# hihixuyang/LQR-Obstacles

Hardware: AMD Instinct MI355X
Metric: agent-pair LQR-obstacle evals/sec (higher is better)
Workload: dtype f64

## Files before the change

lqr-obstacles_amd/csrc/lqro_device.hpp:

```cpp
#pragma once
#include <hip/hip_runtime.h>
#include <stdint.h>

namespace lqro {

constexpr int kWave = 64;

#define LQRO_ROW_BIG (1 << 20)

#define LQRO_ST_PAIRS 0
#define LQRO_ST_PLANES 1
#define LQRO_ST_INSIDE 2
#define LQRO_ST_HULLOK 3
#define LQRO_ST_HULLFAIL 4
#define LQRO_ST_BACKUP 5
#define LQRO_ST_NREACH 6
#define LQRO_ST_GTESTS 7
#define LQRO_ST_MERGED 8
#define LQRO_ST_RETRY 9
#define LQRO_ST_TIMEOUT 10
#define LQRO_ST_NFAIL 11
#define LQRO_ST_MWIN 12
#define LQRO_ST_NBUILD 13
#define LQRO_ST_FAILS 16
// ... 14 lines not shown
  LQRO_HC_HOT = 6,
  LQRO_HC_HOT_NEXT = 7,
  LQRO_HC_UNUSED8 = 8,
  LQRO_HC_LP4 = 9,
  LQRO_HC_LP4_NEXT = 10,
  LQRO_HC_LHAND = 11,
  LQRO_HC_LHAND_NEXT = 12,
  LQRO_HC_LDONE = 13,
  LQRO_HC_UNUSED14 = 14,
  LQRO_HC_FACET0 = 15,
  LQRO_HC_WORDS = 16
};

enum : int {
  LQRO_H2_PREV = 0,
  LQRO_H2_HOT1 = 1,
  LQRO_H2_HOT1_NEXT = 2,
  LQRO_H2_HOT2_NEXT = 3,
  LQRO_H2_HOT2_DONE = 4,
  LQRO_H2_SPEC = 5,
  LQRO_H2_SPEC_NEXT = 6,
  LQRO_H2_UNUSED7 = 7,
  LQRO_H2_WORDS = 8
};

enum : int {
  LQRO_PROF_HULL = 0,
  LQRO_PROF_HJOBS = LQRO_PROF_HULL + 32,
  LQRO_PROF_PAIR = LQRO_PROF_HJOBS + 2 * 4096,
  LQRO_PROF_LFAIL = LQRO_PROF_PAIR + 16 + 16,
  LQRO_PROF_LJOBS = LQRO_PROF_LFAIL + 16,
  LQRO_PROF_QW1 = LQRO_PROF_LJOBS + 4 * 4096,
  LQRO_PROF_QLONG = LQRO_PROF_QW1 + 64,
  LQRO_PROF_WORDS = LQRO_PROF_QLONG + 24 * 1024,
  LQRO_PROF_HULL_WORDS = LQRO_PROF_LFAIL
};

__device__ __forceinline__ int opaque(int x) {
  asm volatile("" : "+v"(x));
  return x;
}

__device__ __forceinline__ double uniform(double v) {
  const long long b = __double_as_longlong(v);
  const int lo = __builtin_amdgcn_readfirstlane((int)b);
  const int hi = __builtin_amdgcn_readfirstlane((int)(b >> 32));
  return __longlong_as_double(((long long)hi << 32) | (unsigned)lo);
}

__device__ __forceinline__ void wave_lds_sync() {
  __builtin_amdgcn_fence(__ATOMIC_RELEASE, "workgroup");
  __builtin_amdgcn_wave_barrier();
  __builtin_amdgcn_fence(__ATOMIC_ACQUIRE, "workgroup");
}

template <int CTRL, int ROWS>
__device__ __forceinline__ int dpp_i(int old, int x) {
  return __builtin_amdgcn_update_dpp(old, x, CTRL, ROWS, 0xF, false);
}
template <int CTRL, int ROWS>
__device__ __forceinline__ double dpp_d(double old, double x) {
  const long long o = __double_as_longlong(old), v = __double_as_longlong(x);
  const int lo = dpp_i<CTRL, ROWS>((int)o, (int)v);
  const int hi = dpp_i<CTRL, ROWS>((int)(o >> 32), (int)(v >> 32));
  return __longlong_as_double(((long long)hi << 32) | (unsigned)lo);
}
__device__ __forceinline__ int wave_incl_scan(int x) {
// ... 107 lines not shown
```

lqr-obstacles_amd/csrc/lqro_plan.hpp:

```cpp
#pragma once

#include <algorithm>
#include <climits>
#include <cstddef>
#include <cstdlib>
#include <vector>

namespace lqro {

struct StepKnobs {
  int hot_on;
  int hot_split;
  int hot_spec;
  long hot_max_inside;
  double hot_t, hot_r;
  int qside;
  int qside_pct;
  int qspare;
  int qbalance;
  int qhull_inline;
  int qhull_big;
  int qhull_flags;
  int hull_big_only;
  int local_hull;
// ... 5 lines not shown

inline int env_int(const char* name, int dflt) {
  const char* e = std::getenv(name);
  return e ? std::atoi(e) : dflt;
}
inline long env_long(const char* name, long dflt) {
  const char* e = std::getenv(name);
  return e ? std::atol(e) : dflt;
}
inline double env_double(const char* name, double dflt) {
  const char* e = std::getenv(name);
  return e ? std::atof(e) : dflt;
}

inline StepKnobs knobs_from_env(int n_cu) {
  StepKnobs k{};
  k.qhull_big = env_int("LQRO_QHULL_BIG", 0) != 0;
  k.side_cus = std::max(0, std::min(n_cu / 2, env_int("LQRO_SIDE_HULL_CUS", (3 * n_cu) / 8)));
  k.hull_big_only = env_int("LQRO_HULL_BIG", 0) != 0;
  k.local_hull = env_int("LQRO_LOCAL_HULL", 1) != 0;
  k.lside_cus = std::max(0, std::min(n_cu / 2, env_int("LQRO_LOCAL_SIDE_CUS", (3 * n_cu) / 16)));
  k.hot_on = env_int("LQRO_HOT", 1) != 0;
  k.hot_t = env_double("LQRO_HOT_T", 3.0);
  k.hot_r = env_double("LQRO_HOT_R", 3.0);
  k.lhull_prof = env_int("LQRO_LHULL_PROFILE", 0) != 0;
  k.hot_max_inside = env_long("LQRO_HOT_MAX_INSIDE", -1L);
  k.early_lp = env_int("LQRO_EARLY_LP", 1) != 0;
  k.hot_split = env_int("LQRO_HOT_SPLIT", 1) != 0;
  k.hot_spec = env_int("LQRO_HOT_SPEC", 1) != 0;
  k.qspare = env_int("LQRO_QHULL_SPARE", 4);
  k.qside_pct = std::max(1, std::min(100, env_int("LQRO_QHULL_SIDE_PCT", 100)));
  k.qside = env_int("LQRO_QSIDE", 0) != 0;
  k.qhull_inline = env_int("LQRO_QHULL_INLINE_BIG", 1) != 0;
  k.qhull_flags = env_int("LQRO_QHULL_FLAGS", 119);
  k.qbalance = env_int("LQRO_QHULL_BALANCE", 1) != 0;
  return k;
}

struct StepFeedback {
  unsigned long long inside;
  unsigned long long sweep_work;
  unsigned long long build_work;
  unsigned long long build_max;
  unsigned long long retried;
  unsigned long long unused[3];
};
static_assert(sizeof(StepFeedback) == 8 * sizeof(unsigned long long), "one slot is 8 words");
constexpr StepFeedback kNoFeedback = {~0ull, 0ull, 0ull, 0ull, 0ull, {0ull, 0ull, 0ull}};

struct StepShape {
  int n_cu, nrows;
  int npr;
  int nbr_k;
  size_t hnp;
  int per_agent, qhull_order;
  int phase;
  bool has_newv;
  bool newv_is_callers;
  int waves, lds_wave, wave_doubles;
  size_t hull_lds_max_hnp;
  size_t hull_lds_doubles;
  int hull_cwaves;
  size_t qhull_lds_doubles;
  size_t lp_lds_max;
  int early_lp_max_npr;
  int row_big;
  int extra_planes = 0;
// ... 135 lines not shown
```

lqr-obstacles_amd/csrc/lqro_qh_front.inc:

```
int simplex[4];
{
  int maxpoints[6];
  S.max_outside = 0.0;
  S.MAXabs_coord = 0.0;
  S.MAXwidth = -DBL_MAX;
  S.MAXsumcoord = 0.0;
  for (int k = 0; k < 3; k++) {
    int mn, mx;
    qh_extreme(W.Pr, n, k, false, lane, &mn);
    qh_extreme(W.Pr, n, k, true, lane, &mx);
    const double maxk = W.Pr[3 * (size_t)mx + k], mink = W.Pr[3 * (size_t)mn + k];
    const double maxcoord = fmax(maxk, -mink);
    const double temp = maxk - mink;
    if (temp > S.MAXwidth) S.MAXwidth = temp;
    if (maxcoord > S.MAXabs_coord) S.MAXabs_coord = maxcoord;
    S.MAXsumcoord += maxcoord;
    maxpoints[2 * k] = mn;
    maxpoints[2 * k + 1] = mx;
    S.NEARzero[k] = 80 * S.MAXsumcoord * DBL_EPSILON;
  }
  {
    double maxdistsum = sqrt(3.0) * S.MAXabs_coord;
    if (S.MAXsumcoord < maxdistsum) maxdistsum = S.MAXsumcoord;
    S.DISTround = DBL_EPSILON * (3 * maxdistsum * 1.01 + S.MAXabs_coord);
    const double MINdenom_1 = fmax(1.0 / DBL_MAX, DBL_MIN);
    S.MINdenom = MINdenom_1 * S.MAXabs_coord;
    S.MINdenom_2 = sqrt(MINdenom_1 * 3) * S.MAXabs_coord;
    S.MINvisible = 0.0 + 2 * S.DISTround;
    S.MAXcoplanar = S.MINvisible;
    S.MINoutside = 2 * S.MINvisible;
  }
  {
    double maxcoord = -DBL_MAX, mincoord = DBL_MAX;
    int minx = -1, maxx = -1;
    for (int i = 0; i < 6; i++) {
      const double c = W.Pr[3 * (size_t)maxpoints[i]];
      if (maxcoord < c) { maxcoord = c; maxx = maxpoints[i]; }
      if (mincoord > c) { mincoord = c; minx = maxpoints[i]; }
    }
    double maxdet = maxcoord - mincoord;
    int ns = 0;
    simplex[ns++] = minx;
    if (maxx != minx) simplex[ns++] = maxx;
    if (ns < 2) { S.status |= QHS_INPUT; QH_FRONT_FAIL; }
    for (int i = 2; i < 4; i++) {
      const double prevdet = maxdet;
      int maxpoint = -1, maxnearzero = 0, nearzero;
      maxdet = -1.0;
      for (int m = 0; m < 6; m++) {
        const int p = maxpoints[m];
        bool ins = false;
        for (int t = 0; t < i; t++) ins |= simplex[t] == p;
        if (!ins && p != maxpoint) {
// ... 30 lines not shown
```

lqr-obstacles_amd/csrc/lqro_qhull3.hpp:

```cpp
#pragma once
#include "lqro_qhull.hpp"
#include "lqro_qhull3_prof.hpp"
#include "lqro_lp.hpp"

namespace lqro {

#ifndef Q3_NEWCAP
#define Q3_NEWCAP 128
#endif
#ifndef Q3_VISCAP
#define Q3_VISCAP 192
#endif
#define Q3_MOVCAP 16
#define Q3_HZCAP 24
#define Q3_COPCAP 8
#define Q3_FSTK 512
#define Q3_ND (Q3_NEWCAP + Q3_MOVCAP)
#define Q3_WAVES 4
#define Q3_HR 4
#ifndef Q3_W0_SLEEP
#define Q3_W0_SLEEP 1
#endif
#ifndef Q3_W1_SLEEP
#define Q3_W1_SLEEP 1
// ... 1686 lines not shown
    int cnt = 0;
    if (vi < nvis) {
      const int f = L.sp_visf[vi];
      cnt = (int)(q3_cc(W, L, f) & 0xffffu) - (vi == 0 ? 1 : 0);
      L.pf_vsoff[vi] = W.soff[f];
      L.pf_vscnt[vi] = cnt;
    }
    np += __builtin_amdgcn_readlane(q3_scan_add(cnt), 63);
  }
  hl_sync();
  if (lane < np) {
    int a = 0, base = 0;
    for (;;) {
      const int k = L.pf_vscnt[a];
      if (lane < base + k || a == nvis - 1) break;
      base += k;
      ++a;
    }
    const int q = W.sb[L.pf_vsoff[a] + lane - base];
    HullPt r;
    r.x = W.Pr[3 * (size_t)q]; r.y = W.Pr[3 * (size_t)q + 1]; r.z = W.Pr[3 * (size_t)q + 2];
    r.q = q;
    r.pad = 0;
    L.pf_pre[lane] = r;
    L.pf_prea[lane] = (unsigned char)a;
  }
  hl_sync();
  if (lane == 0) {
    L.pf_np = np;
    q3_st_rel(&L.pf_done, p);
  }
}

__device__ inline void q3_build(const Q3W& W, Q3S& S, Q3L& L, int n, int lane) {
#ifdef LQRO_QHULL_PROFILE
  S.pf.tq = __builtin_amdgcn_s_memtime();
#endif
  const unsigned long long ltmask = (1ull << lane) - 1ull;
  S.status = 0;
  S.nalloc = 1;
  S.nfs = 0;
  S.sbtop = 0;
  S.nnew = S.nvis = S.nmov = S.nold = 0;
  S.findbestnew = S.notsharp = 0;
  S.hgen = 0;
  S.egen = 0;
  S.keyc = 1;
  S.key0_last = 0;
  S.qhead = S.qtail = 0;
  if (W.FC > 65535) {
    S.status |= QHS_CAPACITY | Q3_CAPBIT(QHS_CAP_FACETS);
    return;
  }
#define QH_FRONT_FAIL return
#include "lqro_qh_front.inc"
#undef QH_FRONT_FAIL
  const int pset[4] = {simplex[3], simplex[2], simplex[1], simplex[0]};
  int fs[4];
  {
    int top = 1, tops[4];
    for (int i = 0; i < 4; i++) {
      fs[i] = S.nalloc++;
      tops[i] = top;
      top ^= 1;
    }
    for (int k = 0; k < 3; k++) {
      double c = 0.0;
      for (int t = 0; t < 4; t++) c += W.Pr[3 * (size_t)pset[t] + k];
      S.interior[k] = c / 4;
    }
    int fv[4][3];
    for (int i = 0; i < 4; i++) {
      int m = 0;
      for (int t = 0; t < 4; t++)
        if (t != i) fv[i][m++] = pset[t];
    }
    int ls = 0;
    double q[4][4];
    bool fl[4];
    q3_plane(S, ls, W.Pr + 3 * (size_t)fv[0][0], W.Pr + 3 * (size_t)fv[0][1], W.Pr + 3 * (size_t)fv[0][2], tops[0],
             q[0], &fl[0]);
    if (q3_distq(q[0], S.interior) > S.DISTround)
      for (int i = 0; i < 4; i++) tops[i] ^= 1;
    bool anyflip = false;
    for (int i = 0; i < 4; i++) {
      q3_plane(S, ls, W.Pr + 3 * (size_t)fv[i][0], W.Pr + 3 * (size_t)fv[i][1], W.Pr + 3 * (size_t)fv[i][2],
               tops[i], q[i], &fl[i]);
      anyflip |= fl[i];
    }
    if (anyflip) ls |= QHS_FLIPPED;
    int nbs[4][3];
    for (int i = 0; i < 4; i++) {
      int m = 0;
      for (int t = 0; t < 4; t++)
        if (t != i) nbs[i][m++] = fs[t];
    }
    double minangle = DBL_MAX;
    for (int i = 0; i < 4; i++)
      for (int t = 0; t < 3; t++) {
        int j = 0;
        for (int u = 0; u < 4; u++)
          if (fs[u] == nbs[i][t]) j = u;
        double angle = 0.0;
        for (int k = 0; k < 3; k++) angle += q[i][k] * q[j][k];
        if (angle < minangle) minangle = angle;
      }
    if (minangle < -0.99999999) ls |= QHS_NARROW;
    S.status |= ls;
    hl_sync();
    if (lane == 0)
      for (int i = 0; i < 4; i++) {
        const int f = fs[i];
        q3_set_facet(W, L, f, q[i], nbs[i][0], nbs[i][1], nbs[i][2],
                     QF_LIVE | (tops[i] ? QF_TOP : 0) | (fl[i] ? QF_FLIPPED : 0));
        q3_set_key(W, L, f, S.keyc + i);
        q3_set_cc(W, L, f, 0u);
        Q3V& v = W.vv[f];
        for (int t = 0; t < 3; t++) {
          for (int k = 0; k < 3; k++) v.p[3 * t + k] = W.Pr[3 * (size_t)fv[i][t] + k];
          v.id[t] = fv[i][t];
        }
      }
    S.keyc += 4;
    hl_sync();
    int np = 0;
    for (int c = 0; c < n; c += 64) {
      const int qi = c + lane;
      const bool ok = qi < n && qi != simplex[0] && qi != simplex[1] && qi != simplex[2] && qi != simplex[3];
      const unsigned long long b = __ballot(ok);
      if (ok) W.pq[np + __popcll(b & ltmask)] = qi;
      np += __popcll(b);
    }
    hl_sync();
    const double distoutside = fmax(2 * S.MINoutside, S.max_outside);
    for (int i = 0; i < 4; i++) {
      const int f = fs[i];
      int cnt = 0;
      const int off = S.sbtop;
      double mx = 0.0, cx = 0.0, cy = 0.0, cz = 0.0;
      int champ = -1, w = 0;
      for (int c = 0; c < np; c += 64) {
        const int pos = c + lane;
        HullPt pt;
        pt.x = pt.y = pt.z = 0.0;
        pt.q = -1;
        pt.pad = 0;
        double d = -DBL_MAX;
        if (pos < np) {
          pt.q = W.pq[pos];
          pt.x = W.Pr[3 * (size_t)pt.q]; pt.y = W.Pr[3 * (size_t)pt.q + 1]; pt.z = W.Pr[3 * (size_t)pt.q + 2];
          const double p[3] = {pt.x, pt.y, pt.z};
          d = q3_distq(q[i], p);
        }
        const bool out = pos < np && d >= distoutside;
        const bool keep = pos < np && !out;
        const unsigned long long bk = __ballot(keep);
        hl_sync();
        if (keep) W.pq[w + __popcll(bk & ltmask)] = pt.q;
        w += __popcll(bk);
        const unsigned long long bo = __ballot(out);
        if (bo) {
          int wpos = -1, wr = 0;
          q3_place(bo, lane, ltmask, d, pt, off, W.SB, cnt, mx, champ, cx, cy, cz, wpos, wr);
          if (wpos >= 0) W.sb[wpos] = wr;
        }
        hl_sync();
      }
      if (cnt) {
        if (off + cnt > W.SB) { S.status |= QHS_CAPACITY | Q3_CAPBIT(QHS_CAP_SB); return; }
        if (lane == 0) {
          W.sb[off + cnt - 1] = champ;
          W.soff[f] = off;
          W.fdist[f] = mx;
          q3_set_cc(W, L, f, (unsigned)cnt | ((unsigned)champ << 16));
        }
        S.sbtop += cnt;
      }
      np = w;
      hl_sync();
    }
    if (np > 0) {
      S.nnew = 4;
      if (lane == 0)
        for (int i = 0; i < 4; i++) {
          L.nslot[i] = fs[i];
          for (int k = 0; k < 4; k++) L.npl[4 * i + k] = q[i][k];
          L.nflag[i] = q3_fa(W, L, fs[i]);
          L.nn1[i] = L.nn2[i] = 0;
        }
      S.nmov = 0;
      S.findbestnew = 1;
      hl_sync();
      int rg;
      double rd;
      HullPt rpt, pre;
      pre.x = pre.y = pre.z = 0.0;
      pre.q = -1;
      pre.pad = 0;
      q3_locate_seq(W, S, L, np, 0, true, lane, pre, 0, false, rg, rd, rpt);
      q3_emit_seq(W, S, L, np, 0, true, lane, rg, rd, rpt);
      S.findbestnew = 0;
      S.nnew = 0;
      S.nmov = 0;
      hl_sync();
    }
    if (S.status & (QHS_INPUT | QHS_TOPOLOGY | QHS_CAPACITY)) return;
    {
      int order[4] = {fs[0], fs[1], fs[2], fs[3]};
      unsigned kk[4];
      for (int i = 0; i < 4; i++) kk[i] = q3_key(W, L, order[i]);
      for (int a = 0; a < 4; a++)
        for (int b = a + 1; b < 4; b++)
          if (kk[b] < kk[a]) {
            const unsigned tk = kk[a]; kk[a] = kk[b]; kk[b] = tk;
            const int to = order[a]; order[a] = order[b]; order[b] = to;
          }
      int best = -1;
      double bd = -DBL_MAX;
      for (int i = 0; i < 4; i++) {
        const int f = order[i];
        if ((q3_cc(W, L, f) & 0xffffu) && W.fdist[f] > bd) { best = f; bd = W.fdist[f]; }
      }
      hl_sync();
      if (best >= 0) {
        q3_set_key(W, L, best, 0u);
        for (int i = 0; i < 4; i++)
          if (order[i] == best) {
            for (int t = i; t > 0; t--) { order[t] = order[t - 1]; kk[t] = kk[t - 1]; }
            order[0] = best;
            kk[0] = 0;
            break;
          }
      }
      int qt = 0;
      for (int i = 0; i < 4; i++)
        if (q3_cc(W, L, order[i]) & 0xffffu) {
          if (lane == 0) {
            W.fq[qt] = order[i];
            W.fqk[qt] = kk[i];
            HullPt r;
            r.x = r.y = r.z = 0.0; r.q = -1; r.pad = 0;
            W.fqc[qt] = r;
          }
          qt++;
        }
      S.qhead = 0;
      S.qtail = qt;
      hl_sync();
    }
  }
  Q3T(0);
  if (lane == 0) {
    L.c_dist[0] = S.MINvisible; L.c_dist[1] = S.MAXcoplanar; L.c_dist[2] = S.DISTround;
    L.c_dist[3] = S.MINdenom; L.c_dist[4] = S.MINdenom_2;
    for (int k = 0; k < 3; k++) { L.c_dist[5 + k] = S.NEARzero[k]; L.c_interior[k] = S.interior[k]; }
  }
  int phase = 0;
  int qcb = 0, qcn = 0;
  int qf = 0, qp = -1;
  unsigned qk = 0;
  double qx = 0.0, qy = 0.0, qz = 0.0;
  for (;;) {
#ifdef LQRO_QHULL_PROFILE
    unsigned long long snap_[21];
    for (int k = 0; k < 21; k++) snap_[k] = S.pf.tph[k];
#endif
    int facet = -1, furthest = -1;
    double apexp[3] = {0.0, 0.0, 0.0};
    bool adopt = false;
    bool pfv = false;
    bool fast = false;
    int nvis = 0, nnew = 0, lm = 0;
    const double* ncb = W.ncoord;
    HullPt pre;
    pre.x = pre.y = pre.z = 0.0;
    pre.q = -1;
    pre.pad = 0;
    int pfa = 0, pfnp = -1;
#ifdef LQRO_QHULL_LONGPROF
    const unsigned long long lp_ta = __builtin_amdgcn_s_memrealtime();
    S.pf.lp_tail += S.pf.lp_tw ? lp_ta - S.pf.lp_tw : 0ull;
#endif
    if (phase > 0) {
#ifdef LQRO_QHULL_PROFILE
      const unsigned long long tw_ = __builtin_amdgcn_s_memtime();
#endif
#ifdef LQRO_QHULL_PROFILE
      int spins_ = 0;
      int dn = q3_ld_acq(&L.sp_done);
// ... 459 lines not shown
        if (d1 >= -2 * S.DISTround || d2 >= -2 * S.DISTround || d3 >= -2 * S.DISTround) lm |= QHS_NONCONVEX;
      };
      if (one) {
        if (my_t >= 0) zero(my_t, P1, P2, PO);
      } else {
        for (int t = lane; t < nnew; t += 64) {
          double p1[3], p2[3], po[3];
          for (int k = 0; k < 3; k++) {
            p1[k] = ncb[9 * t + k]; p2[k] = ncb[9 * t + 3 + k]; po[k] = ncb[9 * t + 6 + k];
          }
          zero(t, p1, p2, po);
        }
      }
    }
    S.status |= qh_wave_or(lm);
    Q3T(4);
    if (S.status & (QHS_TOPOLOGY | QHS_CAPACITY)) return;
    hl_sync();
    if (lane == 0) {
      L.pub_qhead = S.qhead;
      L.pub_qtail = S.qtail;
      L.pub_adopt = adopt ? 1 : 0;
      L.pub_nnew = nnew;
    }
    ++phase;
#ifdef LQRO_QHULL_PROFILE
    if (lane == 0) { L.pub_t = __builtin_amdgcn_s_memtime(); L.pub_r = __builtin_amdgcn_s_memrealtime(); }
    if (S.pf.tseen) { S.pf.tpre += __builtin_amdgcn_s_memtime() - S.pf.tseen; S.pf.npre += 1; }
#endif
#ifdef LQRO_QHULL_LONGPROF
    const unsigned long long lp_t0 = __builtin_amdgcn_s_memrealtime();
    S.pf.lp_adopt += lp_t0 - lp_ta;
    if (lane == 0) L.lp_pubr = lp_t0;
#endif
    if (lane == 0) q3_st_rel(&L.ph, phase);
#ifdef LQRO_QHULL_PROFILE
    if (lane == 0) S.pf.trel += __builtin_amdgcn_s_memtime() - L.pub_t;
#endif
    S.findbestnew = 0;
    S.notsharp = 0;
    S.nmov = 0;
    int np2 = 0;
    for (int c0 = 0; c0 < nvis; c0 += 64) {
      const int vi = c0 + lane;
      const int cnt = vi < nvis ? L.vscnt[vi] : 0;
      const int inc = q3_scan_add(cnt);
      if (vi < nvis) L.vinc[vi] = np2 + inc;
      np2 += __builtin_amdgcn_readlane(inc, 63);
    }
    hl_sync();
    int prestart = 0;
    if (pfv && np2 == pfnp) {
      if (lane < np2) prestart = L.repl[pfa] >= 0 ? L.repl[pfa] : 0;
    } else if (lane < np2) {
      pre = q3_seqpt(W, L, nvis, false, lane, &prestart);
    }
    Q3T(5);
    const int sharp = adopt ? L.sp_sharp : q3_sharpnewfacets(S, L, lane);
    Q3T(20);
    Q3C(21, 1);
    S.nins++;
    Q3C(31, adopt ? 1 : 0);
    Q3C(22, np2);
    if (np2) {
      int rg;
      double rd;
// ... 197 lines not shown
__device__ __attribute__((noinline)) void q3_big_inline(const HullArgs& A, QhL& LB, int slot, unsigned long long tjob,
                                                        int wave) {
#else
__device__ inline void q3_big_inline(const HullArgs& A, QhL& LB, int slot, unsigned long long tjob, int wave) {
#endif
  const int lane = threadIdx.x & 63;
  const int HNP = A.H * A.NP;
  const QhW W = qh_worker(A.qscratch + (size_t)(A.block_base + blockIdx.x) * A.qstride, HNP);
  const HullJob J = hull_job(A, slot);
  const int n = hull_points(A, LB, J.Ti, J.Ni, J.xi, J.xj, J.vrel, W.Pr, W.Pf);
  if (wave == 0) qh_one_job(A, W, LB, J, n, slot, tjob, lane);
}

__device__ __forceinline__ void q3_body(const HullArgs& A, Q3L& L, QhL* LB = nullptr) {
  const int lane = threadIdx.x & 63;
  const int wave = __builtin_amdgcn_readfirstlane(threadIdx.x >> 6);
  const int HNP = A.H * A.NP;
  const Q3W W = q3_worker(A.qscratch + (size_t)(A.block_base + blockIdx.x) * A.qstride, HNP);
  for (;;) {
    const int slot = hull_take_job(A, L, false);
    if (slot < 0) break;
    const unsigned long long tjob = __builtin_amdgcn_s_memrealtime();
    const bool spec = A.spec_mark != nullptr && A.spec_mark[slot] >= 2;
    if (threadIdx.x == 0) {
      L.ph = 0; L.sp_done = 0; L.sp_gdone = 0; L.hctl = 0u; L.hbusy = 0; L.sp_hz = 0; L.pf_done = 0;
      L.ectl = 0u; L.edone = 0;
      L.qflags = A.qflags;
      q3_longprof_begin(L);
      L.big_slot = -1;
    }
    for (int q = threadIdx.x; q < Q3_FL / 2; q += blockDim.x) reinterpret_cast<unsigned*>(L.mark)[q] = 0u;
    const HullJob J = hull_job(A, slot);
    const int n = hull_points(A, L, J.Ti, J.Ni, J.xi, J.xj, J.vrel, W.Pr, W.Pf);
    bool lp_go = false;
    if (wave >= 2) {
      const Q3Col CH = q3_colh(W, wave, lane);
      int last = 0;
      long idle = 0;
      for (;;) {
        if (wave == 2) {
          const int hz = q3_ld_acq(&L.sp_hz);
          if (hz != last && hz > 0) {
            last = hz;
            q3_prefetch(W, L, lane, hz);
            idle = 0;
            continue;
          }
        }
        if (q3_help(W, L, lane, CH)) { idle = 0; continue; }
        if (q3_emit_help(W, L, lane)) { idle = 0; continue; }
        if (q3_ld_acq(&L.ph) < 0) break;
        if (++idle > (1l << 24)) break;
        __builtin_amdgcn_s_sleep(Q3_W2_SLEEP);
      }
    } else if (wave == 1) {
      unsigned* owner = qw_owner(A.qscratch + (size_t)(A.block_base + blockIdx.x) * A.qstride, A.qstride);
      if (*owner != QW_OWNER_Q3) {
        for (int q = lane; q < W.FC; q += 64) W.mark2[q] = 0u;
        if (lane == 0) { W.ctr[0] = 0u; *owner = QW_OWNER_Q3; }
      }
      unsigned ep2 = W.ctr[0];
      unsigned short ep = 0;
      const Q3Col CH = q3_colh(W, 1, lane);
      int last = 0;
      Q3QC Q;
      Q.qcb = 0; Q.qcn = 0; Q.qf = 0; Q.qp = -1; Q.qk = 0u; Q.qx = Q.qy = Q.qz = 0.0;
// ... 37 lines not shown
          if (lane == 0) q3_st_rel(&L.sp_gdone, p);
          if (L.qflags & 4) q3_prescan(W, L, lane, ep, ep2, Q);
#ifdef LQRO_QHULL_PROFILE
          if (lane == 0) { L.done_t2 = __builtin_amdgcn_s_memtime(); L.done_r = __builtin_amdgcn_s_memrealtime(); }
          P.tq2 = __builtin_amdgcn_s_memtime();
          P.t[0] += __builtin_amdgcn_s_memtime() - t0_;
          P.t[7] += 1;
#endif
          idle = 0;
          continue;
        }
        {
#ifdef LQRO_QHULL_PROFILE
          const unsigned long long t0_ = __builtin_amdgcn_s_memtime();
#endif
          if (q3_help(W, L, lane, CH)) {
#ifdef LQRO_QHULL_PROFILE
            P.t[6] += __builtin_amdgcn_s_memtime() - t0_;
            P.t[8] += 1;
#endif
            idle = 0;
            continue;
          }
        }
        if (q3_emit_help(W, L, lane)) { idle = 0; continue; }
        if (++idle > (1l << 24)) break;
        __builtin_amdgcn_s_sleep(Q3_W1_SLEEP);
      }
      q3_prof_w1_flush(A, P, lane);
      if (lane == 0) W.ctr[0] = ep2;
    } else {
    Q3S S;
    q3_prof_begin(S.pf);
    S.status = 0;
    S.nalloc = 1;
    S.nins = 0;
    if (L.fail || n < 4) S.status = QHS_INPUT;
    else q3_build(W, S, L, n, lane);
    hl_sync();
    if (lane == 0) q3_st_rel(&L.ph, -1);
    bool keep = true;
    if (spec) {
      int m = 0;
      if (lane == 0) {
        m = __hip_atomic_load(A.spec_mark + slot, __ATOMIC_ACQUIRE, __HIP_MEMORY_SCOPE_AGENT);
        for (long w = 0; m == 2 && w < (1l << 26); ++w) {
          __builtin_amdgcn_s_sleep(8);
          m = __hip_atomic_load(A.spec_mark + slot, __ATOMIC_ACQUIRE, __HIP_MEMORY_SCOPE_AGENT);
        }
        if (m == 2) {
          atomicAdd(&A.stats[LQRO_ST_TIMEOUT], 1ull);
          hull_fail_note(A.stats, slot);
        }
      }
      keep = __builtin_amdgcn_readfirstlane(m) == 3;
    }
    if (!keep) {
    } else if (S.status & QHS_CAPACITY) {
      if (lane == 0) {
        atomicAdd(&A.stats[LQRO_ST_RETRY], 1ull);
        if (S.status & QHS_TIMEOUT) atomicAdd(&A.stats[LQRO_ST_TIMEOUT], 1ull);
        if (LB) {
          L.big_slot = slot;
        } else {
          const int r = atomicAdd(A.rcount, 1);
          if (r < A.cap) A.rqueue[r] = slot;
// ... 46 lines not shown
```

lqr-obstacles_amd/csrc/lqro_qhull3_prof.hpp:

```cpp
#pragma once
#include "lqro_hull_job.hpp"

namespace lqro {

#define Q3_PROF_RETRY (LQRO_PROF_PAIR + 16)
#ifdef LQRO_QHULL_PROFILE
#define Q3_CAPBIT(b) (b)
#else
#define Q3_CAPBIT(b) 0
#endif

struct Q3Prof {
#if defined(LQRO_QHULL_PROFILE) || defined(LQRO_QHULL_LONGPROF)
  unsigned long long tph[32];
  unsigned long long tq;
  unsigned long long tjob;
  unsigned long long tw, nw;
  unsigned long long tdl;
  unsigned long long tw1, nw1;
  unsigned long long tse, tsn;
  unsigned long long tfr, nsp;
  unsigned long long tfr2, trel;
  unsigned long long r_start, r_done, r_seen, r_gseen;
  unsigned long long tseen, tpre, npre, tstart;
  int prev1;
  unsigned long long tps[24], nps;
  unsigned long long lp_n, lp_pts, lp_t, lp_all, lp_tloc, lp_wait, lp_adopt, lp_tail, lp_tw;
  unsigned long long lp_own, lp_got, lp_hwait, lp_stop, lp_ev, lp_posts;
#endif
};

#if defined(LQRO_QHULL_PROFILE) && defined(LQRO_QHULL_PROF_LIGHT)
#define Q3T(k) do { const unsigned long long t_ = __builtin_amdgcn_s_memtime(); S.pf.tph[k] += t_ - S.pf.tq; S.pf.tq = t_; } while (0)
#elif defined(LQRO_QHULL_PROFILE)
#define Q3T(k) do { __builtin_amdgcn_s_waitcnt(0); const unsigned long long t_ = __builtin_amdgcn_s_memtime(); S.pf.tph[k] += t_ - S.pf.tq; S.pf.tq = t_; } while (0)
#else
#define Q3T(k) do {} while (0)
#endif
#define Q3_PROF_W1 LQRO_PROF_QW1
#define Q3_PROF_LONG LQRO_PROF_QLONG
struct Q3P {
  unsigned long long tq2 = 0;
  unsigned long long t[16];
  unsigned long long tq;
};
#if defined(LQRO_QHULL_PROFILE) && defined(LQRO_QHULL_PROF_LIGHT)
#define W1T(k) do { const unsigned long long t_ = __builtin_amdgcn_s_memtime(); P.t[k] += t_ - P.tq; P.tq = t_; } while (0)
#elif defined(LQRO_QHULL_PROFILE)
#define W1T(k) do { __builtin_amdgcn_s_waitcnt(0); const unsigned long long t_ = __builtin_amdgcn_s_memtime(); P.t[k] += t_ - P.tq; P.tq = t_; } while (0)
#else
#define W1T(k) do {} while (0)
#endif
#ifdef LQRO_QHULL_PROFILE
#define Q3C(k, v) do { S.pf.tph[k] += (unsigned long long)(v); } while (0)
#else
#define Q3C(k, v) do {} while (0)
#endif

__device__ __forceinline__ void q3_prof_begin(Q3Prof& F) {
#if defined(LQRO_QHULL_PROFILE) || defined(LQRO_QHULL_LONGPROF)
  F.lp_n = F.lp_pts = F.lp_t = F.lp_all = F.lp_tloc = F.lp_wait = F.lp_adopt = F.lp_tail = F.lp_tw = 0;
  F.lp_own = F.lp_got = F.lp_hwait = F.lp_stop = F.lp_ev = F.lp_posts = 0;
#endif
#ifdef LQRO_QHULL_PROFILE
  for (int k = 0; k < 32; k++) F.tph[k] = 0;
  F.tw = F.nw = 0;
  F.tdl = 0;
  F.tw1 = F.nw1 = 0;
  F.tse = F.tsn = 0;
  F.tfr = F.nsp = 0;
  F.tfr2 = 0;
  F.trel = 0;
  F.r_start = F.r_done = F.r_seen = F.r_gseen = 0;
  F.tseen = F.tpre = F.npre = F.tstart = 0;
  F.prev1 = 0;
  for (int k = 0; k < 24; k++) F.tps[k] = 0;
  F.nps = 0;
  F.tjob = __builtin_amdgcn_s_memtime();
#endif
}

__device__ __forceinline__ void q3_prof_stamp(Q3Prof& F) {
#ifdef LQRO_QHULL_PROFILE
  F.tq = __builtin_amdgcn_s_memtime();
#endif
}

__device__ __forceinline__ void q3_prof_flush(const HullArgs& A, Q3Prof& F, int n, int nalloc, int lane) {
#ifdef LQRO_QHULL_PROFILE
  F.tph[10] = __builtin_amdgcn_s_memtime() - F.tq;
  F.tph[27] = __builtin_amdgcn_s_memtime() - F.tjob;
  F.tph[28] = (unsigned long long)n;
  if (A.prof && lane == 0) {
    for (int k = 0; k < 32; k++)
      if (k != 26 && k != 11) atomicAdd(&A.prof[k], F.tph[k]);
// ... 32 lines not shown
  if (A.prof) {
    const unsigned long long k = atomicAdd(&A.prof[Q3_PROF_RETRY], 1ull);
    atomicOr(&A.prof[Q3_PROF_RETRY + 1], (unsigned long long)status);
    if (k < 14) A.prof[Q3_PROF_RETRY + 2 + k] = (unsigned long long)slot | ((unsigned long long)status << 32);
  }
#endif
}

__device__ __forceinline__ void q3_prof_w1_flush(const HullArgs& A, const Q3P& P, int lane) {
#ifdef LQRO_QHULL_PROFILE
  if (A.prof && lane == 0)
    for (int k = 0; k < 16; k++) atomicAdd(&A.prof[Q3_PROF_W1 + k], P.t[k]);
#endif
}

template <class LT>
__device__ __forceinline__ void q3_longprof_begin(LT& L) {
#ifdef LQRO_QHULL_LONGPROF
  for (int k = 0; k < 12; k++) L.hprof[k] = 0ull;
  L.lp_pubr = L.lp_doner = 0ull;
#endif
}

template <class LT>
__device__ __forceinline__ void q3_longprof_flush(const HullArgs& A, int k, const Q3Prof& F, const LT& L) {
#ifdef LQRO_QHULL_LONGPROF
  if (A.prof && k >= 0 && k < 1024) {
    unsigned long long* r = A.prof + Q3_PROF_LONG + 24 * k;
    r[0] = F.lp_n; r[1] = F.lp_pts; r[2] = F.lp_t; r[3] = F.lp_all;
    r[4] = F.lp_tloc; r[5] = F.lp_wait; r[6] = F.lp_adopt - F.lp_wait; r[7] = F.lp_tail;
    r[8] = F.lp_own; r[9] = F.lp_got; r[10] = F.lp_hwait; r[11] = F.lp_stop; r[12] = F.lp_ev; r[13] = F.lp_posts;
    r[14] = L.hprof[0]; r[15] = L.hprof[1] | (L.hprof[2] << 32);
    for (int q = 3; q < 11; q++) r[13 + q] = L.hprof[q];
  }
#endif
}

}
```

Before: 59.91 million.

## Parallelize qhull initial simplex and outside-set partition across all block waves

Adds a block-wide q3_start routine that finds the six extreme points with a cross-wave reduction, builds the initial simplex facets, and partitions points into per-facet outside sets using every wave in the workgroup. q3_build then adopts the precomputed tolerances, counts and facets instead of doing that work on a single wave. It is enabled through the new default qhull flag bit 8, and profiling stamps are added. It adds extra block barriers and shared scratch use, and the full point set is scanned once per facet.

```diff
diff --git a/lqr-obstacles_amd/csrc/lqro_device.hpp b/lqr-obstacles_amd/csrc/lqro_device.hpp
--- a/lqr-obstacles_amd/csrc/lqro_device.hpp
+++ b/lqr-obstacles_amd/csrc/lqro_device.hpp
@@ -70,7 +70,8 @@
   LQRO_PROF_LJOBS = LQRO_PROF_LFAIL + 16,
   LQRO_PROF_QW1 = LQRO_PROF_LJOBS + 4 * 4096,
   LQRO_PROF_QLONG = LQRO_PROF_QW1 + 64,
-  LQRO_PROF_WORDS = LQRO_PROF_QLONG + 24 * 1024,
+  LQRO_PROF_QSTART = LQRO_PROF_QLONG + 24 * 1024,
+  LQRO_PROF_WORDS = LQRO_PROF_QSTART + 12 * 1024,
   LQRO_PROF_HULL_WORDS = LQRO_PROF_LFAIL
 };
 
diff --git a/lqr-obstacles_amd/csrc/lqro_plan.hpp b/lqr-obstacles_amd/csrc/lqro_plan.hpp
--- a/lqr-obstacles_amd/csrc/lqro_plan.hpp
+++ b/lqr-obstacles_amd/csrc/lqro_plan.hpp
@@ -61,7 +61,7 @@
   k.qside_pct = std::max(1, std::min(100, env_int("LQRO_QHULL_SIDE_PCT", 100)));
   k.qside = env_int("LQRO_QSIDE", 0) != 0;
   k.qhull_inline = env_int("LQRO_QHULL_INLINE_BIG", 1) != 0;
-  k.qhull_flags = env_int("LQRO_QHULL_FLAGS", 119);
+  k.qhull_flags = env_int("LQRO_QHULL_FLAGS", 127);
   k.qbalance = env_int("LQRO_QHULL_BALANCE", 1) != 0;
   return k;
 }
diff --git a/lqr-obstacles_amd/csrc/lqro_qh_front.inc b/lqr-obstacles_amd/csrc/lqro_qh_front.inc
--- a/lqr-obstacles_amd/csrc/lqro_qh_front.inc
+++ b/lqr-obstacles_amd/csrc/lqro_qh_front.inc
@@ -19,6 +19,9 @@
     maxpoints[2 * k + 1] = mx;
     S.NEARzero[k] = 80 * S.MAXsumcoord * DBL_EPSILON;
   }
+#ifdef QH_FRONT_MAXMIN_DONE
+  QH_FRONT_MAXMIN_DONE;
+#endif
   {
     double maxdistsum = sqrt(3.0) * S.MAXabs_coord;
     if (S.MAXsumcoord < maxdistsum) maxdistsum = S.MAXsumcoord;
diff --git a/lqr-obstacles_amd/csrc/lqro_qhull3.hpp b/lqr-obstacles_amd/csrc/lqro_qhull3.hpp
--- a/lqr-obstacles_amd/csrc/lqro_qhull3.hpp
+++ b/lqr-obstacles_amd/csrc/lqro_qhull3.hpp
@@ -1742,6 +1742,232 @@
   }
 }
 
+struct Q3StL {
+  double key[Q3_WAVES][6];
+  int idx[Q3_WAVES][6];
+  int cnt[Q3_WAVES][5];
+  int status;
+  int np, sbtop;
+  int pad;
+  QhTol tol;
+#ifdef LQRO_QHULL_LONGPROF
+  unsigned long long stamp[4];
+#endif
+};
+static_assert(sizeof(Q3StL) <= sizeof(double) * Q3_HR * 64, "q3_start's words fit the helpers' result buffer");
+#ifdef LQRO_QHULL_LONGPROF
+#define Q3STL(k) do { if (threadIdx.x == 0) T.stamp[k] = __builtin_amdgcn_s_memrealtime(); } while (0)
+#else
+#define Q3STL(k) do {} while (0)
+#endif
+
+__device__ __forceinline__ bool q3_start_front(const Q3W& W, Q3S& S, int n, int lane, const int* ext6, int* sx) {
+#define QH_FRONT_FAIL return false
+#define qh_extreme(Pr_, n_, k_, max_, lane_, out_) (*(out_) = ext6[2 * (k_) + ((max_) ? 1 : 0)])
+#include "lqro_qh_front.inc"
+#undef qh_extreme
+#undef QH_FRONT_FAIL
+  for (int i = 0; i < 4; i++) sx[i] = simplex[i];
+  return true;
+}
+
+__device__ inline void q3_start(const Q3W& W, Q3L& L, int n, int lane, int wave) {
+  if (L.fail || n < 4 || W.FC > 65535) return;
+  Q3StL& T = *reinterpret_cast<Q3StL*>(L.hr_d);
+  const unsigned long long ltmask = (1ull << lane) - 1ull;
+  const int nw = (int)(blockDim.x >> 6);
+  int ext6[6];
+  {
+    double key[6];
+    int idx[6];
+    for (int m = 0; m < 6; m++) { key[m] = -DBL_MAX; idx[m] = 0x7fffffff; }
+    for (int q = wave * 64 + lane; q < n; q += 64 * nw)
+      for (int k = 0; k < 3; k++) {
+        const double c = W.Pr[3 * (size_t)q + k];
+        const double v0 = -c, v1 = c;
+        if (v0 > key[2 * k] || (v0 == key[2 * k] && q < idx[2 * k])) { key[2 * k] = v0; idx[2 * k] = q; }
+        if (v1 > key[2 * k + 1] || (v1 == key[2 * k + 1] && q < idx[2 * k + 1])) { key[2 * k + 1] = v1; idx[2 * k + 1] = q; }
+      }
+    for (int m = 0; m < 6; m++) {
+      for (int off = 32; off >= 1; off >>= 1) {
+        const double ok = __shfl_xor(key[m], off);
+        const int oi = __shfl_xor(idx[m], off);
+        if (ok > key[m] || (ok == key[m] && oi < idx[m])) { key[m] = ok; idx[m] = oi; }
+      }
+      if (lane == 0) { T.key[wave][m] = key[m]; T.idx[wave][m] = idx[m]; }
+    }
+    hl_bar();
+    for (int m = 0; m < 6; m++) {
+      double bk = T.key[0][m];
+      int bi = T.idx[0][m];
+      for (int w = 1; w < nw; w++) {
+        const double ok = T.key[w][m];
+        const int oi = T.idx[w][m];
+        if (ok > bk || (ok == bk && oi < bi)) { bk = ok; bi = oi; }
+      }
+      ext6[m] = bi;
+    }
+  }
+  Q3STL(0);
+  Q3S S;
+  S.status = 0;
+  int sx[4];
+  const bool ok = q3_start_front(W, S, n, lane, ext6, sx);
+  const int pset[4] = {sx[3], sx[2], sx[1], sx[0]};
+  double q[4][4];
+  double distoutside = 0.0;
+  if (ok) {
+    int top = 1, tops[4];
+    for (int i = 0; i < 4; i++) {
+      tops[i] = top;
+      top ^= 1;
+    }
+    for (int k = 0; k < 3; k++) {
+      double c = 0.0;
+      for (int t = 0; t < 4; t++) c += W.Pr[3 * (size_t)pset[t] + k];
+      S.interior[k] = c / 4;
+    }
+    int fv[4][3];
+    for (int i = 0; i < 4; i++) {
+      int m = 0;
+      for (int t = 0; t < 4; t++)
+        if (t != i) fv[i][m++] = pset[t];
+    }
+    int ls = 0;
+    bool fl[4];
+    q3_plane(S, ls, W.Pr + 3 * (size_t)fv[0][0], W.Pr + 3 * (size_t)fv[0][1], W.Pr + 3 * (size_t)fv[0][2], tops[0],
+             q[0], &fl[0]);
+    if (q3_distq(q[0], S.interior) > S.DISTround)
+      for (int i = 0; i < 4; i++) tops[i] ^= 1;
+    bool anyflip = false;
+    for (int i = 0; i < 4; i++) {
+      q3_plane(S, ls, W.Pr + 3 * (size_t)fv[i][0], W.Pr + 3 * (size_t)fv[i][1], W.Pr + 3 * (size_t)fv[i][2],
+               tops[i], q[i], &fl[i]);
+      anyflip |= fl[i];
+    }
+    if (anyflip) ls |= QHS_FLIPPED;
+    double minangle = DBL_MAX;
+    for (int i = 0; i < 4; i++)
+      for (int j = 0; j < 4; j++) {
+        if (j == i) continue;
+        double angle = 0.0;
+        for (int k = 0; k < 3; k++) angle += q[i][k] * q[j][k];
+        if (angle < minangle) minangle = angle;
+      }
+    if (minangle < -0.99999999) ls |= QHS_NARROW;
+    S.status |= ls;
+    if (wave == 0 && lane == 0)
+      for (int i = 0; i < 4; i++) {
+        const int f = 1 + i;
+        int nb[3], m = 0;
+        for (int t = 0; t < 4; t++)
+          if (t != i) nb[m++] = 1 + t;
+        q3_set_facet(W, L, f, q[i], nb[0], nb[1], nb[2], QF_LIVE | (tops[i] ? QF_TOP : 0) | (fl[i] ? QF_FLIPPED : 0));
+        q3_set_key(W, L, f, 1u + i);
+        q3_set_cc(W, L, f, 0u);
+        Q3V& v = W.vv[f];
+        for (int t = 0; t < 3; t++) {
+          for (int k = 0; k < 3; k++) v.p[3 * t + k] = W.Pr[3 * (size_t)fv[i][t] + k];
+          v.id[t] = fv[i][t];
+        }
+      }
+    distoutside = fmax(2 * S.MINoutside, S.max_outside);
+  }
+  Q3STL(1);
+  const int per = (((n + 63) >> 6) + nw - 1) / nw * 64;
+  const int c0 = wave * per, c1 = min(n, c0 + per);
+  {
+    int cn[5] = {0, 0, 0, 0, 0};
+    if (ok)
+      for (int c = c0; c < c1; c += 64) {
+        const int qi = c + lane;
+        const bool in = qi < c1 && qi != sx[0] && qi != sx[1] && qi != sx[2] && qi != sx[3];
+        int tag = -1;
+        if (in) {
+          const double p[3] = {W.Pr[3 * (size_t)qi], W.Pr[3 * (size_t)qi + 1], W.Pr[3 * (size_t)qi + 2]};
+          tag = 4;
+          for (int i = 3; i >= 0; i--)
+            if (q3_distq(q[i], p) >= distoutside) tag = i;
+        }
+        for (int i = 0; i < 4; i++) cn[i] += __popcll(__ballot(tag == i));
+        const unsigned long long br = __ballot(tag == 4);
+        if (tag == 4) W.pdst[c0 + cn[4] + __popcll(br & ltmask)] = qi;
+        cn[4] += __popcll(br);
+      }
+    if (lane == 0) {
+      for (int i = 0; i < 5; i++) T.cnt[wave][i] = cn[i];
+      if (wave == 0) T.status = S.status;
+    }
+  }
+  hl_bar();
+  Q3STL(2);
+  if (T.status & QHS_INPUT) return;
+  int tot[5], before = 0;
+  for (int i = 0; i < 5; i++) {
+    tot[i] = 0;
+    for (int w = 0; w < nw; w++) tot[i] += T.cnt[w][i];
+  }
+  for (int w = 0; w < wave; w++) before += T.cnt[w][4];
+  const int mine = T.cnt[wave][4];
+  const int sbtop = tot[0] + tot[1] + tot[2] + tot[3];
+  if (sbtop > W.SB) {
+    hl_bar();
+    if (wave == 0 && lane == 0) T.status = S.status | QHS_CAPACITY | Q3_CAPBIT(QHS_CAP_SB);
+    hl_bar();
+    return;
+  }
+  for (int k = lane; k < mine; k += 64) W.pq[before + k] = W.pdst[c0 + k];
+  for (int fi = wave; fi < 4; fi += nw) {
+    int off = 0;
+    double qm[4] = {q[0][0], q[0][1], q[0][2], q[0][3]};
+    for (int i = 1; i < 4; i++)
+      if (fi >= i) {
+        off += tot[i - 1];
+        for (int k = 0; k < 4; k++) qm[k] = q[i][k];
+      }
+    const int f = 1 + fi;
+    int cnt = 0;
+    double mx = 0.0, cx = 0.0, cy = 0.0, cz = 0.0;
+    int champ = -1;
+    double nx = 0.0, ny = 0.0, nz = 0.0;
+    if (lane < n) { nx = W.Pr[3 * (size_t)lane]; ny = W.Pr[3 * (size_t)lane + 1]; nz = W.Pr[3 * (size_t)lane + 2]; }
+    for (int c = 0; c < n; c += 64) {
+      const int qi = c + lane;
+      HullPt pt;
+      pt.x = nx; pt.y = ny; pt.z = nz;
+      pt.q = qi < n ? qi : -1;
+      pt.pad = 0;
+      const int qn = qi + 64;
+      if (qn < n) { nx = W.Pr[3 * (size_t)qn]; ny = W.Pr[3 * (size_t)qn + 1]; nz = W.Pr[3 * (size_t)qn + 2]; }
+      const double p[3] = {pt.x, pt.y, pt.z};
+      bool cand = qi < n && qi != sx[0] && qi != sx[1] && qi != sx[2] && qi != sx[3];
+      for (int i = 0; i < 3; i++)
+        if (i < fi) cand &= !(q3_distq(q[i], p) >= distoutside);
+      const double d = cand ? q3_distq(qm, p) : -DBL_MAX;
+      const bool out = cand && d >= distoutside;
+      const unsigned long long bo = __ballot(out);
+      if (bo) {
+        int wpos = -1, wr = 0;
+        q3_place(bo, lane, ltmask, d, pt, off, W.SB, cnt, mx, champ, cx, cy, cz, wpos, wr);
+        if (wpos >= 0) W.sb[wpos] = wr;
+      }
+    }
+    if (cnt && lane == 0) {
+      W.sb[off + cnt - 1] = champ;
+      W.soff[f] = off;
+      W.fdist[f] = mx;
+      q3_set_cc(W, L, f, (unsigned)cnt | ((unsigned)champ << 16));
+    }
+  }
+  if (wave == 0 && lane == 0) {
+    T.np = tot[4];
+    T.sbtop = sbtop;
+    T.tol = static_cast<const QhTol&>(S);
+  }
+  hl_bar();
+  Q3STL(3);
+}
+
 __device__ inline void q3_build(const Q3W& W, Q3S& S, Q3L& L, int n, int lane) {
 #ifdef LQRO_QHULL_PROFILE
   S.pf.tq = __builtin_amdgcn_s_memtime();
@@ -1762,11 +1988,32 @@
     S.status |= QHS_CAPACITY | Q3_CAPBIT(QHS_CAP_FACETS);
     return;
   }
+  int fs[4];
+  double q[4][4];
+  int np = 0;
+  if (L.qflags & 8) {
+    const Q3StL& T = *reinterpret_cast<const Q3StL*>(L.hr_d);
+    S.status |= T.status;
+    if (S.status & (QHS_INPUT | QHS_CAPACITY)) return;
+    static_cast<QhTol&>(S) = T.tol;
+    for (int i = 0; i < 4; i++) {
+      fs[i] = S.nalloc++;
+      q3_pl(W, L, fs[i], q[i]);
+    }
+    S.keyc += 4;
+    S.sbtop = T.sbtop;
+    np = T.np;
+#ifdef LQRO_QHULL_LONGPROF
+    S.pf.st[2] = T.stamp[0]; S.pf.st[3] = T.stamp[1]; S.pf.st[4] = T.stamp[2];
+    S.pf.st[5] = S.pf.st[6] = S.pf.st[7] = S.pf.st[8] = T.stamp[3];
+#endif
+  } else {
 #define QH_FRONT_FAIL return
+#define QH_FRONT_MAXMIN_DONE Q3ST(2)
 #include "lqro_qh_front.inc"
+#undef QH_FRONT_MAXMIN_DONE
 #undef QH_FRONT_FAIL
   const int pset[4] = {simplex[3], simplex[2], simplex[1], simplex[0]};
-  int fs[4];
   {
     int top = 1, tops[4];
     for (int i = 0; i < 4; i++) {
@@ -1786,7 +2033,6 @@
         if (t != i) fv[i][m++] = pset[t];
     }
     int ls = 0;
-    double q[4][4];
     bool fl[4];
     q3_plane(S, ls, W.Pr + 3 * (size_t)fv[0][0], W.Pr + 3 * (size_t)fv[0][1], W.Pr + 3 * (size_t)fv[0][2], tops[0],
              q[0], &fl[0]);
@@ -1833,7 +2079,8 @@
       }
     S.keyc += 4;
     hl_sync();
-    int np = 0;
+    Q3ST(3);
+    np = 0;
     for (int c = 0; c < n; c += 64) {
       const int qi = c + lane;
       const bool ok = qi < n && qi != simplex[0] && qi != simplex[1] && qi != simplex[2] && qi != simplex[3];
@@ -1842,6 +2089,7 @@
       np += __popcll(b);
     }
     hl_sync();
+    Q3ST(4);
     const double distoutside = fmax(2 * S.MINoutside, S.max_outside);
     for (int i = 0; i < 4; i++) {
       const int f = fs[i];
@@ -1888,6 +2136,18 @@
       }
       np = w;
       hl_sync();
+      Q3ST(5 + i);
+    }
+  }
+  }
+  {
+#ifdef LQRO_QHULL_LONGPROF
+    S.pf.st[11] = (unsigned long long)np;
+#endif
+    if (lane == 0) {
+      L.c_dist[0] = S.MINvisible; L.c_dist[1] = S.MAXcoplanar; L.c_dist[2] = S.DISTround;
+      L.c_dist[3] = S.MINdenom; L.c_dist[4] = S.MINdenom_2;
+      for (int k = 0; k < 3; k++) { L.c_dist[5 + k] = S.NEARzero[k]; L.c_interior[k] = S.interior[k]; }
     }
     if (np > 0) {
       S.nnew = 4;
@@ -1914,6 +2174,7 @@
       S.nmov = 0;
       hl_sync();
     }
+    Q3ST(9);
     if (S.status & (QHS_INPUT | QHS_TOPOLOGY | QHS_CAPACITY)) return;
     {
       int order[4] = {fs[0], fs[1], fs[2], fs[3]};
@@ -1960,11 +2221,6 @@
     }
   }
   Q3T(0);
-  if (lane == 0) {
-    L.c_dist[0] = S.MINvisible; L.c_dist[1] = S.MAXcoplanar; L.c_dist[2] = S.DISTround;
-    L.c_dist[3] = S.MINdenom; L.c_dist[4] = S.MINdenom_2;
-    for (int k = 0; k < 3; k++) { L.c_dist[5 + k] = S.NEARzero[k]; L.c_interior[k] = S.interior[k]; }
-  }
   int phase = 0;
   int qcb = 0, qcn = 0;
   int qf = 0, qp = -1;
@@ -2490,6 +2746,7 @@
     const unsigned long long lp_t0 = __builtin_amdgcn_s_memrealtime();
     S.pf.lp_adopt += lp_t0 - lp_ta;
     if (lane == 0) L.lp_pubr = lp_t0;
+    if (!S.pf.st[10]) S.pf.st[10] = lp_t0;
 #endif
     if (lane == 0) q3_st_rel(&L.ph, phase);
 #ifdef LQRO_QHULL_PROFILE
@@ -2753,6 +3010,10 @@
     for (int q = threadIdx.x; q < Q3_FL / 2; q += blockDim.x) reinterpret_cast<unsigned*>(L.mark)[q] = 0u;
     const HullJob J = hull_job(A, slot);
     const int n = hull_points(A, L, J.Ti, J.Ni, J.xi, J.xj, J.vrel, W.Pr, W.Pf);
+#ifdef LQRO_QHULL_LONGPROF
+    const unsigned long long tpts = __builtin_amdgcn_s_memrealtime();
+#endif
+    if (A.qflags & 8) q3_start(W, L, n, lane, wave);
     bool lp_go = false;
     if (wave >= 2) {
       const Q3Col CH = q3_colh(W, wave, lane);
@@ -2856,6 +3117,10 @@
     } else {
     Q3S S;
     q3_prof_begin(S.pf);
+#ifdef LQRO_QHULL_LONGPROF
+    S.pf.st[0] = tjob;
+    S.pf.st[1] = tpts;
+#endif
     S.status = 0;
     S.nalloc = 1;
     S.nins = 0;
diff --git a/lqr-obstacles_amd/csrc/lqro_qhull3_prof.hpp b/lqr-obstacles_amd/csrc/lqro_qhull3_prof.hpp
--- a/lqr-obstacles_amd/csrc/lqro_qhull3_prof.hpp
+++ b/lqr-obstacles_amd/csrc/lqro_qhull3_prof.hpp
@@ -10,6 +10,7 @@
 #define Q3_CAPBIT(b) 0
 #endif
 
+#define Q3_START_STAMPS 12
 struct Q3Prof {
 #if defined(LQRO_QHULL_PROFILE) || defined(LQRO_QHULL_LONGPROF)
   unsigned long long tph[32];
@@ -27,6 +28,7 @@
   unsigned long long tps[24], nps;
   unsigned long long lp_n, lp_pts, lp_t, lp_all, lp_tloc, lp_wait, lp_adopt, lp_tail, lp_tw;
   unsigned long long lp_own, lp_got, lp_hwait, lp_stop, lp_ev, lp_posts;
+  unsigned long long st[Q3_START_STAMPS];
 #endif
 };
 
@@ -39,6 +41,12 @@
 #endif
 #define Q3_PROF_W1 LQRO_PROF_QW1
 #define Q3_PROF_LONG LQRO_PROF_QLONG
+#define Q3_PROF_START LQRO_PROF_QSTART
+#ifdef LQRO_QHULL_LONGPROF
+#define Q3ST(k) do { S.pf.st[k] = __builtin_amdgcn_s_memrealtime(); } while (0)
+#else
+#define Q3ST(k) do {} while (0)
+#endif
 struct Q3P {
   unsigned long long tq2 = 0;
   unsigned long long t[16];
@@ -61,6 +69,7 @@
 #if defined(LQRO_QHULL_PROFILE) || defined(LQRO_QHULL_LONGPROF)
   F.lp_n = F.lp_pts = F.lp_t = F.lp_all = F.lp_tloc = F.lp_wait = F.lp_adopt = F.lp_tail = F.lp_tw = 0;
   F.lp_own = F.lp_got = F.lp_hwait = F.lp_stop = F.lp_ev = F.lp_posts = 0;
+  for (int k = 0; k < Q3_START_STAMPS; k++) F.st[k] = 0;
 #endif
 #ifdef LQRO_QHULL_PROFILE
   for (int k = 0; k < 32; k++) F.tph[k] = 0;
@@ -159,6 +168,8 @@
     r[8] = F.lp_own; r[9] = F.lp_got; r[10] = F.lp_hwait; r[11] = F.lp_stop; r[12] = F.lp_ev; r[13] = F.lp_posts;
     r[14] = L.hprof[0]; r[15] = L.hprof[1] | (L.hprof[2] << 32);
     for (int q = 3; q < 11; q++) r[13 + q] = L.hprof[q];
+    unsigned long long* s = A.prof + Q3_PROF_START + Q3_START_STAMPS * k;
+    for (int q = 0; q < Q3_START_STAMPS; q++) s[q] = F.st[q];
   }
 #endif
 }
```

After: 59.91 million. Within noise of the previous version (-0.0%).
